# Rose-STL-Lab/spherical-dyffusion

Measured on AMD Instinct MI355X. Metric: forecast-steps/sec (180x360, 63ch), 25-member ensemble DYffusion sampling, whole job, higher is better.
Workload: dtype f32 tensors; every GEMM-class kernel (1x1 convs, fused MLP, Legendre analysis/synthesis, dhconv) as 3-pass split-f16 MFMA with f32 accumulation; FFT / norms / pointwise in f32 (statistics f64)

## Files before the change

### spherical-dyffusion_amd/csrc/conv_h3.hip

```cpp
#include <cmath>
#include <cstdlib>
#include <type_traits>
#include <vector>

#include "common.h"

namespace {

constexpr int CE = 256;
constexpr int CTN = 64;
constexpr int CKMAX = 384;
constexpr int CRING = 4;
constexpr float CSX = SDY_ACT_SX;
constexpr int CSTAT_BYTES = CE * 2 * 8;
#ifndef SDY_CONV_STAMP_T0
#define SDY_CONV_STAMP_T0 2
#endif

template <int KBLK, int NW>
struct ConvCfg {
  static_assert(NW == 4 || NW == 8, "4 or 8 waves");
  static constexpr int NT = 64 * NW;
  static constexpr int MT = 8 / NW;
  static constexpr int RS = 4 * NW;
  static constexpr int OC = (8 * KBLK + RS - 1) / RS;
  static constexpr int RPT = 64 / NW;
  static constexpr int PPI = (8 * OC + RPT - 1) / RPT;
  static constexpr int KROW = KBLK <= 4 ? 256 : 384;
  static constexpr int KSW = KROW / 16;
  static constexpr int GPK = 4 * MT;
  static constexpr int GPW = MT * KSW;
  static constexpr int WGS = NW == 4 ? 2 : 1;
  static constexpr int TILE_BYTES = 2 * CTN * KROW * 2;
  static constexpr int LDS_BYTES = TILE_BYTES + CSTAT_BYTES + CE * 4 + SDY_GELU_TAB_BYTES;
};
#ifndef SDY_CONV_GELU_TAB
#define SDY_CONV_GELU_TAB 1
#endif

struct ConvParams {
  const float* x; long x_bs;
  const float* pa; const float* pd;
  const sdy_f16x8* w;
  const float* bias;
  const float* add; long add_bs; int add_mode;
  int act;
  float* out; long out_bs;
  int out_tiled;
  double* stats;
  int HW, B;
  int Cin;
  float out_scale;
  unsigned* flags;
  unsigned* head;
  const float* gelu_tab;
  SdyImgMap xmap;
  unsigned long long* stamps;
};

__device__ __forceinline__ int cv_swz(int px) { return (px & 15) ^ (((px >> 4) & 1) * 3); }
template <int KROW>
__device__ __forceinline__ int cv_off(int px, int c) { return px * KROW + (((c & ~15) | ((c ^ cv_swz(px)) & 15)) << 3); }

template <int KBLK, int NW>
__global__ __launch_bounds__(64 * NW, NW == 4 ? 2 : 1) void conv_h3_kernel(const ConvParams p) {
  using G = ConvCfg<KBLK, NW>;
  constexpr int CMT = G::MT, CRS = G::RS, COC = G::OC, CRPT = G::RPT, KROW = G::KROW, CGPK = G::GPK, CGPW = G::GPW;
  __shared__ __attribute__((aligned(16))) unsigned char smem[G::LDS_BYTES];
  _Float16* Xs_hi = reinterpret_cast<_Float16*>(smem);
  _Float16* Xs_lo = Xs_hi + CTN * KROW;
  float* Os = reinterpret_cast<float*>(smem);

  const int tid = threadIdx.x, lane = tid & 63, wave = tid >> 6;
  int h = lane >> 5, l31 = lane & 31;
  int q0 = tid & 15, o0 = tid >> 4;
  const int tpi = (p.HW + CTN - 1) / CTN;
  const int ntiles = tpi * p.B;
  const int t_per = (ntiles + (int)gridDim.x - 1) / (int)gridDim.x;
  const int t_begin = (int)blockIdx.x * t_per;
  const int t_end = (t_begin + t_per < ntiles) ? t_begin + t_per : ntiles;

  sdy_f16x8 r_hi[CRING], r_lo[CRING];
  constexpr int CGROUP_BYTES = SDY_GROUP * (int)sizeof(sdy_f16x8);
  const char* const wbase = reinterpret_cast<const char*>(p.w) + (size_t)__builtin_amdgcn_readfirstlane(wave) * CGPW * CGROUP_BYTES;
  unsigned woff = (unsigned)lane * 16u;
#pragma unroll
  for (int s = 0; s < CRING; ++s) {
    r_hi[s] = sdy_ring_ld(wbase, woff, 0);
    r_lo[s] = sdy_ring_ld(wbase, woff, CGROUP_BYTES / 2);
    woff += CGROUP_BYTES;
  }
  constexpr int NWIN = KBLK * CMT;
  if (NWIN == 1) woff -= CRING * CGROUP_BYTES;

  double* Ss = reinterpret_cast<double*>(smem + G::TILE_BYTES);
  float* Bs = reinterpret_cast<float*>(smem + G::TILE_BYTES + CSTAT_BYTES);
  if (tid < CE) {
    Bs[tid] = p.bias ? p.bias[tid] / p.out_scale : 0.0f;
    Ss[2 * tid] = 0.0; Ss[2 * tid + 1] = 0.0;
  }
  float* Gt = reinterpret_cast<float*>(smem + G::TILE_BYTES + CSTAT_BYTES + CE * 4);
  const unsigned gt_base = (unsigned)(uintptr_t)Gt;
  const bool tab_gelu = SDY_CONV_GELU_TAB && p.act == 1;
  if (tab_gelu) gelu_tab_to_lds(Gt, p.gelu_tab, tid, G::NT, 1.0f / SDY_GELU_SX);
  const float os_scale = tab_gelu ? p.out_scale * SDY_GELU_WS : p.out_scale;

  f32x4 xr[COC][8], addv[CRPT];
  auto img = [&](const float* base, long bs, int t) { return base + (long)(t / tpi) * bs; };
  auto ximg = [&](int t) { return p.x + (long)sdy_img(p.xmap, t / tpi) * p.x_bs; };
  auto lane_col = [&](int t) {
    const int nn = (t % tpi) * CTN + 4 * q0;
    return nn < p.HW ? nn : 0;
  };
  const float* addsrc = p.add ? p.add : p.out;
  const long addsrc_bs = p.add ? p.add_bs : p.out_bs;
  if (t_begin < t_end) {
    const float* xz = ximg(t_begin);
    const unsigned xo = (unsigned)(8 * o0 * p.HW + lane_col(t_begin)) * 4u;
#pragma unroll
    for (int oc = 0; oc < COC; ++oc)
#pragma unroll
      for (int e = 0; e < 8; ++e) {
        const int ch = 8 * (o0 + CRS * oc) + e;
        xr[oc][e] = f32x4{0.f, 0.f, 0.f, 0.f};
        if (ch < p.Cin) xr[oc][e] = sdy_ld16s(xz + (long)(8 * CRS * oc + e) * p.HW, xo);
      }
  }

  for (int tile = t_begin; tile < t_end; ++tile) {
    asm volatile("" : "+v"(l31), "+v"(h), "+v"(q0), "+v"(o0));
    const int tile_it = tile - t_begin;
    auto stamp = [&](int i) {
      if (SDY_STAMPS_ON && p.stamps && blockIdx.x == 3 && tid == 0 && tile_it >= SDY_CONV_STAMP_T0 && tile_it < SDY_CONV_STAMP_T0 + 4)
        p.stamps[(tile_it - SDY_CONV_STAMP_T0) * 8 + i] = __builtin_amdgcn_s_memtime();
    };
    stamp(0);
    const int z = tile / tpi;
    const int zx = sdy_img(p.xmap, z);
    const int n0 = (tile - z * tpi) * CTN;
    const bool full = n0 + CTN <= p.HW;

    {
      float amax = 0.0f;
      const bool ok = full || (n0 + 4 * q0 < p.HW);
#pragma unroll
      for (int oc = 0; oc < COC; ++oc) {
        const int c0 = 8 * (o0 + CRS * oc);
        if (8 * CRS * oc + 8 * CRS > KROW && c0 >= KROW) continue;
        float av[8], dv[8];
        if (p.pa) {
          const f32x4 a0 = *reinterpret_cast<const f32x4*>(p.pa + (long)zx * CE + c0);
          const f32x4 a1 = *reinterpret_cast<const f32x4*>(p.pa + (long)zx * CE + c0 + 4);
          const f32x4 d0 = *reinterpret_cast<const f32x4*>(p.pd + (long)zx * CE + c0);
          const f32x4 d1 = *reinterpret_cast<const f32x4*>(p.pd + (long)zx * CE + c0 + 4);
#pragma unroll
          for (int e = 0; e < 4; ++e) {
            av[e] = a0[e] * CSX; av[e + 4] = a1[e] * CSX;
            dv[e] = d0[e] * CSX; dv[e + 4] = d1[e] * CSX;
          }
        } else {
#pragma unroll
          for (int e = 0; e < 8; ++e) { av[e] = CSX; dv[e] = 0.f; }
        }
#pragma unroll
        for (int pp = 0; pp < 4; ++pp) {
          sdy_f16x8 vh, vl;
          float v[8];
#pragma unroll
          for (int e = 0; e < 8; ++e) v[e] = (ok && c0 + e < p.Cin) ? fmaf(xr[oc][e][pp], av[e], dv[e]) : 0.0f;
          sdy_split8(v, vh, vl, amax);
          const int off = cv_off<KROW>(4 * q0 + pp, o0 + CRS * oc);
          *reinterpret_cast<sdy_f16x8*>(Xs_hi + off) = vh;
          *reinterpret_cast<sdy_f16x8*>(Xs_lo + off) = vl;
        }
      }
      sdy_flag_range(p.flags, amax, p.head);
    }
    __syncthreads();
    stamp(1);
    const int col = n0 + 4 * q0;
    const bool c_ok = full || col < p.HW;
    const unsigned ro = (unsigned)(o0 * p.HW + (c_ok ? col : 0)) * 4u;
    const unsigned ro_out = p.out_tiled ? (unsigned)(o0 * CTN + 4 * q0) * 4u : ro;
    const int out_rs = p.out_tiled ? CTN : p.HW;
    const int tnext = (tile + 1 < t_end) ? tile + 1 : tile;
    const float* xz_next = ximg(tnext);
    const unsigned xo_next = (unsigned)(8 * o0 * p.HW + lane_col(tnext)) * 4u;
    stamp(2);
    f32x16 acc[CMT][2];
#pragma unroll
    for (int mi = 0; mi < CMT; ++mi)
#pragma unroll
      for (int r4 = 0; r4 < 4; ++r4) {
        const f32x4 b4 = *reinterpret_cast<const f32x4*>(Bs + 32 * (CMT * wave + mi) + 8 * r4 + 4 * h);
#pragma unroll
        for (int j = 0; j < 2; ++j)
#pragma unroll
          for (int r = 0; r < 4; ++r) acc[mi][j][4 * r4 + r] = b4[r];
      }
#pragma unroll
    for (int kb = 0; kb < KBLK; ++kb) {
#pragma unroll
      for (int i = 0; i < 4; ++i) {
        const int ks = 4 * kb + i;
        sdy_f16x8 bh[2], bl[2];
#pragma unroll
        for (int j = 0; j < 2; ++j) {
          const int off = cv_off<KROW>(32 * j + l31, 2 * ks + h);
          bh[j] = *reinterpret_cast<const sdy_f16x8*>(Xs_hi + off);
          bl[j] = *reinterpret_cast<const sdy_f16x8*>(Xs_lo + off);
        }
#pragma unroll
        for (int mi = 0; mi < CMT; ++mi) {
          const int g = kb * CGPK + CMT * i + mi;
          const int s = g % CRING;
#pragma unroll
          for (int j = 0; j < 2; ++j) SDY_CROSS_TERM(acc[mi][j] = __builtin_amdgcn_mfma_f32_32x32x16_f16(r_lo[s], bh[j], acc[mi][j], 0, 0, 0));
#pragma unroll
          for (int j = 0; j < 2; ++j) SDY_CROSS_TERM(acc[mi][j] = __builtin_amdgcn_mfma_f32_32x32x16_f16(r_hi[s], bl[j], acc[mi][j], 0, 0, 0));
#pragma unroll
          for (int j = 0; j < 2; ++j) acc[mi][j] = __builtin_amdgcn_mfma_f32_32x32x16_f16(r_hi[s], bh[j], acc[mi][j], 0, 0, 0);
          r_hi[s] = sdy_ring_ld(wbase, woff, 0);
          r_lo[s] = sdy_ring_ld(wbase, woff, CGROUP_BYTES / 2);
          woff += CGROUP_BYTES;
          if ((g + CRING + 1) % (NWIN * CRING) == 0) woff -= NWIN * CRING * CGROUP_BYTES;
          __builtin_amdgcn_sched_barrier(0);
        }
      }
    }

    stamp(3);
    {
      const float* az = img(addsrc, addsrc_bs, tile);
#pragma unroll
      for (int i = 0; i < CRPT; ++i) addv[i] = p.add ? sdy_ld16s(az + (long)(CRS * i) * p.HW, ro) : f32x4{0.f, 0.f, 0.f, 0.f};
    }
    __syncthreads();
    stamp(4);
#pragma unroll
    for (int mi = 0; mi < CMT; ++mi)
#pragma unroll
      for (int j = 0; j < 2; ++j)
#pragma unroll
        for (int r = 0; r < 16; ++r) {
          const int row = 32 * (CMT * wave + mi) + (r & 3) + 8 * (r >> 2) + 4 * h;
          Os[row * CTN + 32 * j + l31] = acc[mi][j][r] * os_scale;
        }
    __syncthreads();
    stamp(5);
    {
      float* oz = p.out + (long)z * p.out_bs + (p.out_tiled ? (long)(tile - z * tpi) * (CE * CTN) : 0L);
#pragma unroll
      for (int i = 0; i < CRPT; ++i) {
        f32x4 v = *reinterpret_cast<const f32x4*>(Os + (o0 + CRS * i) * CTN + 4 * q0);
        if (tab_gelu) {
          if (p.add_mode == 1) v = addv[i] * SDY_GELU_WS + v;
          v = f32x4{gelu_tab16(v.x, gt_base), gelu_tab16(v.y, gt_base), gelu_tab16(v.z, gt_base), gelu_tab16(v.w, gt_base)};
        } else {
        if (p.add_mode == 1) v += addv[i];
        if (p.act == 1) {
          const sdy_gf2 g0 = gelu_erf2(sdy_gf2{v.x, v.y}), g1 = gelu_erf2(sdy_gf2{v.z, v.w});
          v = f32x4{g0.x, g0.y, g1.x, g1.y};
        }
        }
        if (p.add_mode == 2) v += addv[i];
        if (c_ok) sdy_st16s(oz + (long)(CRS * i) * out_rs, ro_out, v);
#pragma unroll
        for (int k = 0; k < G::PPI; ++k) {
          const int piece = G::PPI * i + k, oc = piece >> 3, e = piece & 7;
          if (oc < COC) {
            const int ch = 8 * (o0 + CRS * oc) + e;
            if (ch < p.Cin) xr[oc][e] = sdy_ld16s(xz_next + (long)(8 * CRS * oc + e) * p.HW, xo_next);
          }
        }
        if (p.stats) {
          const float s1 = row16_sum(c_ok ? (v.x + v.y) + (v.z + v.w) : 0.0f);
          const float s2 = row16_sum(c_ok ? (v.x * v.x + v.y * v.y) + (v.z * v.z + v.w * v.w) : 0.0f);
          if (q0 == 0) {
            double* st = Ss + 2 * (o0 + CRS * i);
            __hip_atomic_fetch_add(st, (double)s1, __ATOMIC_RELAXED, __HIP_MEMORY_SCOPE_WORKGROUP);
            __hip_atomic_fetch_add(st + 1, (double)s2, __ATOMIC_RELAXED, __HIP_MEMORY_SCOPE_WORKGROUP);
          }
        }
      }
    }
    stamp(6);
    {
      const int nt = tile + 1;
      if (p.stats && (nt >= t_end || nt / tpi != z)) {
        __syncthreads();
        if (tid < CE) {
          double* st = p.stats + ((long)z * CE + tid) * 2;
          __hip_atomic_fetch_add(st, Ss[2 * tid], __ATOMIC_RELAXED, __HIP_MEMORY_SCOPE_AGENT);
          __hip_atomic_fetch_add(st + 1, Ss[2 * tid + 1], __ATOMIC_RELAXED, __HIP_MEMORY_SCOPE_AGENT);
          Ss[2 * tid] = 0.0; Ss[2 * tid + 1] = 0.0;
        }
      }
    }
    stamp(7);
    __syncthreads();
  }
}

}

#if SDY_STAMPS_ON
static unsigned long long* g_cstamps = nullptr;
SDY_DEBUG_EXPORT int sdy_conv256_h3_debug_stamps(unsigned long long* host64) {
  if (!g_cstamps || !host64) return SDY_ERR_STATE;
  SDY_HIP_TRY(hipDeviceSynchronize());
  SDY_HIP_TRY(hipMemcpy(host64, g_cstamps, 64 * sizeof(unsigned long long), hipMemcpyDeviceToHost));
  return SDY_OK;
}
#endif

extern "C" int sdy_conv256_h3_supported(int Cin, int Cout) { return (Cin >= 1 && Cin <= CKMAX && Cout == CE) ? 1 : 0; }

static void conv_layout(int Cin, int* nw, int* ksw, int* mt) {
  const int kblk = (Cin + 63) / 64;
  *nw = kblk <= 4 ? 4 : 8;
  *ksw = kblk <= 4 ? 16 : 24;
  *mt = 8 / *nw;
}

extern "C" size_t sdy_conv256_h3_pack_bytes_cin(int Cin) {
  int nw, ksw, mt;
  conv_layout(Cin < 1 ? 1 : Cin, &nw, &ksw, &mt);
  return (size_t)nw * mt * ksw * SDY_GROUP * sizeof(sdy_f16x8);
}
extern "C" size_t sdy_conv256_h3_pack_bytes(void) { return sdy_conv256_h3_pack_bytes_cin(CE); }

extern "C" int sdy_conv256_h3_pack_cin(const float* w_host, int Cin, void* dev, float* scale) {
  if (!w_host || !dev || !scale || Cin < 1 || Cin > CKMAX) return SDY_ERR_ARG;
  const float s = sdy_h3_scale(sdy_h3_absmax(w_host, (size_t)CE * Cin));
  int nw, ksw, mt;
  conv_layout(Cin, &nw, &ksw, &mt);
  const size_t gh = (size_t)SDY_GROUP * 8;
  std::vector<_Float16> buf((size_t)nw * mt * ksw * gh);
  _Float16* d = buf.data();
  for (int w = 0; w < nw; ++w)
    for (int ks = 0; ks < ksw; ++ks)
      for (int mi = 0; mi < mt; ++mi, d += gh)
        sdy_h3_put_group(d, s, [&](int r, int k) {
          const int kk = 16 * ks + k;
          return kk < Cin ? w_host[(size_t)(32 * (mt * w + mi) + r) * Cin + kk] : 0.0f;
        });
  SDY_HIP_TRY(hipMemcpy(dev, buf.data(), buf.size() * sizeof(_Float16), hipMemcpyHostToDevice));
  *scale = s;
  return SDY_OK;
}
extern "C" int sdy_conv256_h3_pack(const float* w_host, void* dev, float* scale) {
  return sdy_conv256_h3_pack_cin(w_host, CE, dev, scale);
}

template <int KBLK, int NW>
static void conv_launch(const ConvParams& p, long ntiles, int n_cu, hipStream_t stream) {
  using G = ConvCfg<KBLK, NW>;
  const long want = (long)n_cu * G::WGS;
  dim3 grid((unsigned)(ntiles < want ? ntiles : want));
  hipLaunchKernelGGL((conv_h3_kernel<KBLK, NW>), grid, dim3(G::NT), 0, stream, p);
}

int sdy_conv256_h3_launch(const sdy_conv_args* a, hipStream_t stream) {
  if (!a || !a->x || !a->w_frag || !a->out || a->B <= 0 || a->HW <= 0) return SDY_ERR_ARG;
  if (!sdy_conv256_h3_supported(a->Cin, a->Cout)) return SDY_ERR_UNSUPPORTED;
  if (a->drop_p > 0.f || a->keep_mask || a->batch_scale) return SDY_ERR_UNSUPPORTED;
  if (a->pa && a->Cin != CE) return SDY_ERR_UNSUPPORTED;
  if ((a->HW & 3) || (a->x_bstride & 3) || (a->out_bstride & 3) || (a->add_mode && (a->add_bstride & 3))) return SDY_ERR_ALIGN;
  if ((long)a->HW * CKMAX * 4 >= (1L << 32)) return SDY_ERR_UNSUPPORTED;
  ConvParams p;
  p.x = a->x; p.x_bs = a->x_bstride; p.pa = a->pa; p.pd = a->pd;
  p.w = reinterpret_cast<const sdy_f16x8*>(a->w_frag);
  p.bias = a->bias;
  p.add = a->add_mode ? a->add : nullptr; p.add_bs = a->add_bstride; p.add_mode = a->add_mode;
  p.act = a->act;
  p.out = a->out; p.out_bs = a->out_bstride; p.out_tiled = a->out_tiled;
  if (a->out_tiled && a->add_mode && a->add == a->out) return SDY_ERR_ARG;
  p.stats = a->stats;
  SDY_TRY(sdy_flags_ptr(&p.flags));
  SDY_TRY(sdy_headroom_ptr(SDY_RANGE_CONV, &p.head));
  SDY_TRY(sdy_gelu_table_ptr(&p.gelu_tab));
  p.HW = a->HW; p.B = a->B; p.Cin = a->Cin;
  SDY_TRY(sdy_img_map_fill(p.xmap, a->x_rows, a->B));
  p.out_scale = 1.0f / (a->w_frag_scale * CSX);
  p.stamps = nullptr;
#if SDY_STAMPS_ON
  if (std::getenv("SDY_CONV_STAMPS")) {
    if (!g_cstamps) SDY_HIP_TRY(hipMalloc(&g_cstamps, 64 * sizeof(unsigned long long)));
    p.stamps = g_cstamps;
  }
#endif
  int n_cu = 0;
  SDY_TRY(sdy_cu_count(&n_cu));
  const long ntiles = (long)((a->HW + CTN - 1) / CTN) * a->B;
  switch ((a->Cin + 63) / 64) {
    case 1: conv_launch<1, 4>(p, ntiles, n_cu, stream); break;
    case 2: conv_launch<2, 4>(p, ntiles, n_cu, stream); break;
    case 3: conv_launch<3, 4>(p, ntiles, n_cu, stream); break;
    case 4: conv_launch<4, 4>(p, ntiles, n_cu, stream); break;
    case 5: conv_launch<5, 8>(p, ntiles, n_cu, stream); break;
    default: conv_launch<6, 8>(p, ntiles, n_cu, stream); break;
  }
  return sdy_launch_status();
}
```

### spherical-dyffusion_amd/ops.py

```python
from __future__ import annotations

import ctypes as C
from typing import Optional

import torch

from ._lib import SdyConvArgs, SdyMlpArgs, SdyPairArgs, aligned, check, current_stream, lib, ptr


def _f32c(t: torch.Tensor) -> torch.Tensor:
    if not t.is_cuda:
        raise RuntimeError("sdy_amd ops run on the GPU only (no CPU fallback)")
    return aligned(t.to(torch.float32).contiguous())


def _aux(t: torch.Tensor, dev) -> torch.Tensor:
    return t.detach().to(dev, torch.float32).contiguous()


def contract_dhconv(x: torch.Tensor, weight: torch.Tensor, separable: bool = False,
                    operator_type: str = "dhconv", gemm_mode: Optional[str] = None) -> torch.Tensor:
    if separable or operator_type != "dhconv":
        raise NotImplementedError("only the non-separable dhconv contraction is on the hot path")
    B, Ci, L, M = x.shape
    Co = weight.shape[1]
    assert weight.shape == (Ci, Co, L, 2), f"weight shape {tuple(weight.shape)}"
    mtr = min(M, L)
    xr = torch.view_as_real(x.to(torch.complex64).contiguous())
    cs_in = xr[:, :, :, :mtr].permute(2, 3, 0, 4, 1).contiguous()
    cs_out = torch.zeros(L, mtr, B, 2, Co, dtype=torch.float32, device=x.device)
    w_host = weight.detach().to(torch.float32).cpu().contiguous()
    from ._lib import default_gemm_mode
    with torch.cuda.device(x.device):
        mode = gemm_mode or default_gemm_mode()
        if mode == "h3" and lib.sdy_dhconv_frag_supported(Ci, Co):
            wp = torch.empty(lib.sdy_dhconv_frag_pack_bytes(L), dtype=torch.uint8, device=x.device)
            sc = C.c_float()
            check(lib.sdy_dhconv_frag_pack(ptr(w_host), L, ptr(wp), C.byref(sc)), "sdy_dhconv_frag_pack")
            check(lib.sdy_dhconv_frag(ptr(cs_in), ptr(wp), sc.value, ptr(cs_out), L, mtr, B, current_stream()),
                  "sdy_dhconv_frag")
        elif mode == "h3":
            wp = torch.empty(lib.sdy_dhconv_h3_pack_bytes(Ci, Co, L), dtype=torch.uint8, device=x.device)
            sc = C.c_float()
            check(lib.sdy_dhconv_h3_pack_weight(ptr(w_host), Ci, Co, L, ptr(wp), C.byref(sc)), "sdy_dhconv_h3_pack_weight")
            check(lib.sdy_dhconv_h3(ptr(cs_in), ptr(wp), sc.value, ptr(cs_out), L, mtr, B, Ci, Co, current_stream()),
                  "sdy_dhconv_h3")
        else:
            wp = torch.empty(L * 2 * Ci * Co, dtype=torch.float32, device=x.device)
            check(lib.sdy_dhconv_pack_weight(ptr(w_host), Ci, Co, L, ptr(wp), current_stream()), "sdy_dhconv_pack_weight")
            check(lib.sdy_dhconv(ptr(cs_in), ptr(wp), ptr(cs_out), L, mtr, B, Ci, Co, current_stream()), "sdy_dhconv")
    out = torch.zeros(B, Co, L, M, 2, dtype=torch.float32, device=x.device)
    out[:, :, :, :mtr] = cs_out.permute(2, 4, 0, 1, 3)
    tri = (torch.arange(M, device=x.device)[None, :] <= torch.arange(L, device=x.device)[:, None])
    out = out * tri[None, None, :, :, None]
    return torch.view_as_complex(out.contiguous())


def instnorm_coeffs(x: torch.Tensor, gamma: torch.Tensor, beta: torch.Tensor,
                    scale_shift: Optional[torch.Tensor] = None, eps: float = 1e-6):
    x = _f32c(x)
    B, Cc, H, W = x.shape
    a = torch.empty(B, Cc, dtype=torch.float32, device=x.device)
    d = torch.empty_like(a)
    g, b_ = _aux(gamma, x.device), _aux(beta, x.device)
    ss = _aux(scale_shift, x.device) if scale_shift is not None else None
    with torch.cuda.device(x.device):
        check(lib.sdy_instnorm_coeffs(ptr(x), B, Cc, H * W, ptr(g), ptr(b_), ptr(ss), 2 * Cc, eps, ptr(a), ptr(d),
                                      current_stream()), "sdy_instnorm_coeffs")
    return a, d


def conv1x1(x: torch.Tensor, weight: torch.Tensor, bias: Optional[torch.Tensor] = None, *,
            pre_affine=None, add: Optional[torch.Tensor] = None, add_mode: int = 0, gelu: bool = False,
            drop_p: float = 0.0, keep_mask: Optional[torch.Tensor] = None, seed: int = 0, call: int = 0,
            stream_id: int = 0, batch_offset: int = 0, batch_scale: Optional[torch.Tensor] = None,
            kernel_tag: int = 0, out: Optional[torch.Tensor] = None, wt_prepared=None, h3: bool = False,
            h3_prepared=None, frag_prepared=None, stats: Optional[torch.Tensor] = None) -> torch.Tensor:
    x = _f32c(x)
    B, Cin, H, W = x.shape
    w2 = weight.detach().to(torch.float32).reshape(weight.shape[0], -1)
    Cout = w2.shape[0]
    assert w2.shape[1] == Cin
    ldw = (Cout + 3) // 4 * 4
    if wt_prepared is not None:
        wt = wt_prepared
    else:
        wt = torch.zeros(Cin, ldw, dtype=torch.float32, device=x.device)
        wt[:, :Cout] = w2.t().to(x.device)
    if out is None:
        out = torch.empty(B, Cout, H, W, dtype=torch.float32, device=x.device)
    a = SdyConvArgs()
    a.x, a.x_bstride = ptr(x), Cin * H * W
    a.wt, a.ldw = ptr(wt), ldw
    a.out, a.out_bstride = ptr(out), Cout * H * W
    a.B, a.Cin, a.Cout, a.HW = B, Cin, Cout, H * W
    keep = [x, wt, out]
    if h3 or h3_prepared is not None:
        if h3_prepared is None:
            h3_prepared = pack_h3(w2, x.device)
        a.w_h3, a.w_h3_scale = ptr(h3_prepared[0]), h3_prepared[1]
        keep.append(h3_prepared[0])
    if pre_affine is not None:
        pa, pd = _aux(pre_affine[0], x.device), _aux(pre_affine[1], x.device)
        a.pa, a.pd = ptr(pa), ptr(pd)
        keep += [pa, pd]
    if bias is not None:
        bb = _aux(bias, x.device)
        a.bias = ptr(bb)
        keep.append(bb)
    if add is not None:
        ad = _aux(add, x.device)
        a.add = ptr(ad)
        a.add_bstride = 0 if ad.shape[0] == 1 and B > 1 else Cout * H * W
        a.add_mode = add_mode
        keep.append(ad)
    a.act = 1 if gelu else 0
    a.drop_p = drop_p
    if keep_mask is not None:
        km = _aux(keep_mask, x.device)
        a.keep_mask = ptr(km)
        keep.append(km)
    a.seed, a.call, a.stream_id, a.batch_offset = seed, call, stream_id, batch_offset
    a.kernel_tag = kernel_tag
    if frag_prepared is not None:
        a.w_frag, a.w_frag_scale = ptr(frag_prepared[0]), frag_prepared[1]
        keep.append(frag_prepared[0])
    if stats is not None:
        assert stats.dtype == torch.float64 and stats.is_cuda and stats.is_contiguous() and stats.numel() == B * Cout * 2
        a.stats = ptr(stats)
    if batch_scale is not None:
        bs = _aux(batch_scale, x.device)
        a.batch_scale = ptr(bs)
        keep.append(bs)
    with torch.cuda.device(x.device):
        check(lib.sdy_conv1x1(C.byref(a), current_stream()), "sdy_conv1x1")
    return out


def pack_conv256(weight: torch.Tensor, device):
    w = weight.detach().to("cpu", torch.float32).reshape(weight.shape[0], -1).contiguous()
    if not lib.sdy_conv256_h3_supported(w.shape[1], w.shape[0]):
        raise NotImplementedError("the persistent conv kernel needs 256 output and at most 384 input channels")
    buf = torch.empty(lib.sdy_conv256_h3_pack_bytes_cin(w.shape[1]), dtype=torch.uint8, device=device)
    sc = C.c_float()
    with torch.cuda.device(device):
        check(lib.sdy_conv256_h3_pack_cin(ptr(w), w.shape[1], ptr(buf), C.byref(sc)), "sdy_conv256_h3_pack_cin")
    return buf, sc.value


def pack_h3(weight: torch.Tensor, device):
    w = weight.detach().to("cpu", torch.float32).reshape(weight.shape[0], -1).contiguous()
    Cout, Cin = w.shape
    nbytes = lib.sdy_h3_pack_bytes(Cout, Cin)
    buf = torch.empty(nbytes, dtype=torch.uint8, device=device)
    sc = C.c_float()
    with torch.cuda.device(device):
        check(lib.sdy_h3_pack_weight(ptr(w), Cout, Cin, ptr(buf), C.byref(sc)), "sdy_h3_pack_weight")
    return buf, sc.value


def pack_mlp_h3(w1: torch.Tensor, w2: torch.Tensor, device):
    a = w1.detach().to("cpu", torch.float32).reshape(w1.shape[0], -1).contiguous()
    b = w2.detach().to("cpu", torch.float32).reshape(w2.shape[0], -1).contiguous()
    hidden, E = a.shape
    assert b.shape == (E, hidden)
    if not lib.sdy_mlp_h3_supported(E, hidden):
        raise NotImplementedError(f"fused MLP kernel supports E=256, hidden=512 (got {E}, {hidden}); use conv1x1")
    buf = torch.empty(lib.sdy_mlp_h3_pack_bytes(E, hidden), dtype=torch.uint8, device=device)
    s1, s2 = C.c_float(), C.c_float()
    with torch.cuda.device(device):
        check(lib.sdy_mlp_h3_pack(ptr(a), ptr(b), E, hidden, ptr(buf), C.byref(s1), C.byref(s2)), "sdy_mlp_h3_pack")
    return (buf, s1.value, s2.value)


def mlp_fused(x: torch.Tensor, w1: torch.Tensor, b1: torch.Tensor, w2: torch.Tensor, b2: torch.Tensor, *,
              pre_affine=None, add: Optional[torch.Tensor] = None, drop_p: float = 0.0, seed: int = 0, call: int = 0,
              stream_fc1: int = 0, stream_fc2: int = 1, batch_offset: int = 0,
              batch_scale: Optional[torch.Tensor] = None, out: Optional[torch.Tensor] = None,
              prepared=None, add_affine=None, stats: Optional[torch.Tensor] = None,
              keep_masks=None) -> torch.Tensor:
    x = _f32c(x)
    B, E, H, W = x.shape
    if prepared is None:
        prepared = pack_mlp_h3(w1, w2, x.device)
    hidden = b1.numel()
    if out is None:
        out = torch.empty_like(x)
    a = SdyMlpArgs()
    a.x, a.x_bstride = ptr(x), E * H * W
    a.w, a.w1_scale, a.w2_scale = ptr(prepared[0]), prepared[1], prepared[2]
    bb1, bb2 = _aux(b1, x.device), _aux(b2, x.device)
    a.b1, a.b2 = ptr(bb1), ptr(bb2)
    a.out, a.out_bstride = ptr(out), E * H * W
    keep = [x, bb1, bb2, out, prepared]
    if pre_affine is not None:
        pa, pd = _aux(pre_affine[0], x.device), _aux(pre_affine[1], x.device)
        a.pa, a.pd = ptr(pa), ptr(pd)
        keep += [pa, pd]
    if add is not None:
        ad = _aux(add, x.device)
        a.add, a.add_bstride = ptr(ad), E * H * W
        keep.append(ad)
        if add_affine is not None:
            ra, rd = _aux(add_affine[0], x.device), _aux(add_affine[1], x.device)
            a.add_a, a.add_d = ptr(ra), ptr(rd)
            keep += [ra, rd]
    a.B, a.E, a.hidden, a.HW = B, E, hidden, H * W
    a.drop_p = drop_p
    a.seed, a.call, a.stream_fc1, a.stream_fc2, a.batch_offset = seed, call, stream_fc1, stream_fc2, batch_offset
    if batch_scale is not None:
        bs = _aux(batch_scale, x.device)
        a.batch_scale = ptr(bs)
        keep.append(bs)
    if stats is not None:
        assert stats.dtype == torch.float64 and stats.is_cuda and stats.is_contiguous() and stats.numel() == B * E * 2
        a.stats = ptr(stats)
    if keep_masks is not None:
        kh, ko = _aux(keep_masks[0], x.device), _aux(keep_masks[1], x.device)
        assert kh.numel() == B * hidden * H * W and ko.numel() == B * E * H * W
        a.keep_hidden, a.keep_out = ptr(kh), ptr(ko)
        keep += [kh, ko]
    with torch.cuda.device(x.device):
        check(lib.sdy_mlp_h3(C.byref(a), current_stream()), "sdy_mlp_h3")
    return out


def pack_pair_h3(w1: torch.Tensor, w2: torch.Tensor, device):
    a = w1.detach().to("cpu", torch.float32).reshape(w1.shape[0], -1).contiguous()
    b = w2.detach().to("cpu", torch.float32).reshape(w2.shape[0], -1).contiguous()
    hidden, Cin = a.shape
    Cout = b.shape[0]
    assert b.shape == (Cout, hidden)
    if not lib.sdy_pair_h3_supported(Cin, hidden, Cout):
        raise NotImplementedError(f"fused conv pair supports hidden=256 with (Cin<=144, Cout=256) or (Cin<=416, Cout<=64); "
                                  f"got {Cin}->{hidden}->{Cout}; use conv1x1 twice")
    buf = torch.empty(lib.sdy_pair_h3_pack_bytes(Cin, hidden, Cout), dtype=torch.uint8, device=device)
    s1, s2 = C.c_float(), C.c_float()
    with torch.cuda.device(device):
        check(lib.sdy_pair_h3_pack(ptr(a), ptr(b), Cin, hidden, Cout, ptr(buf), C.byref(s1), C.byref(s2)), "sdy_pair_h3_pack")
    return (buf, s1.value, s2.value)


def conv_pair(x: torch.Tensor, w1: torch.Tensor, b1: Optional[torch.Tensor], w2: torch.Tensor, *,
              add: Optional[torch.Tensor] = None, out: Optional[torch.Tensor] = None, prepared=None,
              stats: Optional[torch.Tensor] = None) -> torch.Tensor:
    x = _f32c(x)
    B, Cin, H, W = x.shape
    if prepared is None:
        prepared = pack_pair_h3(w1, w2, x.device)
    hidden, Cout = w1.shape[0], w2.shape[0]
    if out is None:
        out = torch.empty(B, Cout, H, W, dtype=torch.float32, device=x.device)
    a = SdyPairArgs()
    a.x, a.x_bstride = ptr(x), Cin * H * W
    a.w, a.w1_scale, a.w2_scale = ptr(prepared[0]), prepared[1], prepared[2]
    keep = [x, out, prepared]
    if b1 is not None:
        bb1 = _aux(b1, x.device)
        a.b1 = ptr(bb1)
        keep.append(bb1)
    a.out, a.out_bstride = ptr(out), Cout * H * W
    if add is not None:
        ad = _aux(add, x.device)
        a.add, a.add_bstride = ptr(ad), (0 if ad.shape[0] == 1 and B > 1 else Cout * H * W)
        keep.append(ad)
    a.B, a.Cin, a.hidden, a.Cout, a.HW = B, Cin, hidden, Cout, H * W
    if stats is not None:
        assert stats.dtype == torch.float64 and stats.is_cuda and stats.is_contiguous() and stats.numel() == B * Cout * 2
        a.stats = ptr(stats)
    with torch.cuda.device(x.device):
        check(lib.sdy_pair_h3(C.byref(a), current_stream()), "sdy_pair_h3")
    return out


def instnorm_from_stats(stats: torch.Tensor, HW: int, gamma: torch.Tensor, beta: torch.Tensor, scale_shift=None,
                        eps: float = 1e-6):
    B, Cc = stats.shape[0], stats.shape[1]
    dev = stats.device
    g, b_ = _aux(gamma, dev), _aux(beta, dev)
    ss = _aux(scale_shift, dev) if scale_shift is not None else None
    a = torch.empty(B, Cc, dtype=torch.float32, device=dev)
    d = torch.empty(B, Cc, dtype=torch.float32, device=dev)
    with torch.cuda.device(dev):
        check(lib.sdy_instnorm_from_stats(ptr(stats), B, Cc, HW, ptr(g), ptr(b_), ptr(ss), 2 * Cc if ss is not None else 0,
                                          eps, ptr(a), ptr(d), current_stream()), "sdy_instnorm_from_stats")
    return a, d


def cold_update(x_s: torch.Tensor, x_ip_next: torch.Tensor, x_ip_s: Optional[torch.Tensor]) -> torch.Tensor:
    a, b = _f32c(x_s), _f32c(x_ip_next)
    c = _f32c(x_ip_s) if x_ip_s is not None else None
    out = torch.empty_like(a)
    with torch.cuda.device(a.device):
        check(lib.sdy_cold_update(ptr(a), ptr(b), ptr(c), ptr(out), a.numel(), current_stream()), "sdy_cold_update")
    return out


def concat_channels(tensors) -> torch.Tensor:
    ts = [_f32c(t) for t in tensors]
    if len(ts) == 1:
        return ts[0]
    assert 1 <= len(ts) <= 4
    B, _, H, W = ts[0].shape
    chans = [t.shape[1] for t in ts]
    out = torch.empty(B, sum(chans), H, W, dtype=torch.float32, device=ts[0].device)
    srcs = (C.c_void_p * len(ts))(*[ptr(t) for t in ts])
    ch = (C.c_int * len(ts))(*chans)
    with torch.cuda.device(out.device):
        check(lib.sdy_concat_channels(srcs, ch, len(ts), ptr(out), B, H * W, current_stream()), "sdy_concat_channels")
    return out


FLAG_NONFINITE, FLAG_F16_RANGE = 1, 2


def status_flags(reset: bool = True, device=None) -> int:
    dev = torch.device("cuda", torch.cuda.current_device()) if device is None else torch.device(device)
    out = C.c_uint(0)
    with torch.cuda.device(dev):
        check(lib.sdy_status_flags(C.byref(out), 1 if reset else 0, current_stream()), "sdy_status_flags")
    return int(out.value)


RANGE_CLASSES = ("conv_h3 x tile", "mlp_h3 x tile", "dh_h3 coefficient rows", "Legendre analysis input (at rfft360's stores)",
                 "Legendre synthesis input (at dh_h3's stores)")


class range_headroom:

    LIMIT = 65504.0

    def __enter__(self):
        buf = (C.c_float * len(RANGE_CLASSES))()
        with torch.cuda.device(torch.cuda.current_device()):
            check(lib.sdy_range_headroom(buf, 1, current_stream()), "sdy_range_headroom")
        check(lib.sdy_range_headroom_enable(1))
        self.max_staged, self.factor = {}, {}
        return self

    def __exit__(self, *exc):
        check(lib.sdy_range_headroom_enable(0))
        buf = (C.c_float * len(RANGE_CLASSES))()
        with torch.cuda.device(torch.cuda.current_device()):
            check(lib.sdy_range_headroom(buf, 1, current_stream()), "sdy_range_headroom")
        self.max_staged = {n: float(buf[i]) for i, n in enumerate(RANGE_CLASSES)}
        self.factor = {n: (self.LIMIT / v if v > 0.0 else float("inf")) for n, v in self.max_staged.items()}
        return False


def raise_on_status_flags(flags: int, where: str) -> None:
    if not flags:
        return
    why = []
    if flags & FLAG_F16_RANGE:
        why.append("an activation exceeded the fp16 range of the split-precision kernels (|value| * 16 >= 65504, i.e. "
                   "|value| >= 4094 after normalisation)")
    if flags & FLAG_NONFINITE:
        why.append("an InstanceNorm statistic came out inf / NaN (a tensor inside the network holds non-finite values)")
    from ._lib import SdyError
    raise SdyError(f"{where}: " + "; ".join(why) + ".  Inputs are expected standardised; if the data really need the range, "
                   "run the fp32-MFMA path: SDY_GEMM_MODE=f32 (or gemm_mode='f32').")


class stage_timer:

    def __enter__(self):
        n = lib.sdy_profile_stage_count()
        check(lib.sdy_profile_read((C.c_double * n)(), (C.c_long * n)(), n))
        check(lib.sdy_profile_enable(1))
        self.stages, self.rows = {}, {}
        return self

    def __exit__(self, *exc):
        check(lib.sdy_profile_enable(0))
        n = lib.sdy_profile_stage_count()
        ms, cnt, rows = (C.c_double * n)(), (C.c_long * n)(), (C.c_long * n)()
        check(lib.sdy_profile_read_rows(ms, cnt, rows, n), "sdy_profile_read_rows")
        self.stages = {lib.sdy_profile_stage_name(i).decode(): (int(cnt[i]), float(ms[i])) for i in range(n) if cnt[i]}
        self.rows = {lib.sdy_profile_stage_name(i).decode(): int(rows[i]) for i in range(n) if cnt[i]}
        return False
```

Baseline: 162.5.

## Split conv K-staging and epilogue into halves to fit three workgroups per CU

Sets the 4-wave conv kernel's occupancy target to 3 workgroups per CU and halves the LDS x-tile. The input is staged and consumed in two K halves with a barrier between them, and the fp32 epilogue is written out in two row halves. This cuts LDS footprint and register pressure so more waves can hide latency. In exchange it adds extra barriers and serialises staging against the MFMA work within a tile. The Python wrapper also gains out_tiled and x_rows options.

```diff
diff --git a/spherical-dyffusion_amd/csrc/conv_h3.hip b/spherical-dyffusion_amd/csrc/conv_h3.hip
--- a/spherical-dyffusion_amd/csrc/conv_h3.hip
+++ b/spherical-dyffusion_amd/csrc/conv_h3.hip
@@ -13,6 +13,9 @@
 constexpr int CRING = 4;
 constexpr float CSX = SDY_ACT_SX;
 constexpr int CSTAT_BYTES = CE * 2 * 8;
+#ifndef SDY_CONV_WGS
+#define SDY_CONV_WGS 3
+#endif
 #ifndef SDY_CONV_STAMP_T0
 #define SDY_CONV_STAMP_T0 2
 #endif
@@ -25,13 +28,21 @@
   static constexpr int RS = 4 * NW;
   static constexpr int OC = (8 * KBLK + RS - 1) / RS;
   static constexpr int RPT = 64 / NW;
-  static constexpr int PPI = (8 * OC + RPT - 1) / RPT;
   static constexpr int KROW = KBLK <= 4 ? 256 : 384;
   static constexpr int KSW = KROW / 16;
   static constexpr int GPK = 4 * MT;
   static constexpr int GPW = MT * KSW;
-  static constexpr int WGS = NW == 4 ? 2 : 1;
-  static constexpr int TILE_BYTES = 2 * CTN * KROW * 2;
+  static constexpr int WGS = NW == 4 ? SDY_CONV_WGS : 1;
+  static constexpr int NSP = WGS >= 3 ? 2 : 1;
+  static_assert(NSP == 1 || (NSP == MT && KROW == 256 && RS == KROW / 8 / NSP), "halves = the staging role's octet sets");
+  static constexpr int KH = KROW / NSP;
+  static constexpr int KBH = KROW / 64 / NSP;
+  static constexpr int NKH = (KBLK + KBH - 1) / KBH;
+  static constexpr int RPR = RPT / NSP;
+  static constexpr int PPI = (8 * OC + RPT - 1) / RPT;
+  static constexpr int row_c(int rd, int i) { return NSP == 1 ? RS * i : 32 * (MT * ((RS * i) >> 5) + rd) + ((RS * i) & 31); }
+  static constexpr int TILE_BYTES = 2 * CTN * KH * 2;
+  static_assert(CE / NSP * CTN * 4 <= TILE_BYTES, "the epilogue's fp32 staging aliases the x tile");
   static constexpr int LDS_BYTES = TILE_BYTES + CSTAT_BYTES + CE * 4 + SDY_GELU_TAB_BYTES;
 };
 #ifndef SDY_CONV_GELU_TAB
@@ -58,22 +69,36 @@
   unsigned long long* stamps;
 };
 
+__device__ __forceinline__ float sdy_uniform(float v) {
+  return __builtin_bit_cast(float, __builtin_amdgcn_readfirstlane(__builtin_bit_cast(int, v)));
+}
 __device__ __forceinline__ int cv_swz(int px) { return (px & 15) ^ (((px >> 4) & 1) * 3); }
 template <int KROW>
 __device__ __forceinline__ int cv_off(int px, int c) { return px * KROW + (((c & ~15) | ((c ^ cv_swz(px)) & 15)) << 3); }
 
 template <int KBLK, int NW>
-__global__ __launch_bounds__(64 * NW, NW == 4 ? 2 : 1) void conv_h3_kernel(const ConvParams p) {
+__global__ __launch_bounds__(64 * NW, NW == 4 ? SDY_CONV_WGS : 1) void conv_h3_kernel(const ConvParams p) {
   using G = ConvCfg<KBLK, NW>;
-  constexpr int CMT = G::MT, CRS = G::RS, COC = G::OC, CRPT = G::RPT, KROW = G::KROW, CGPK = G::GPK, CGPW = G::GPW;
+  constexpr int CMT = G::MT, CRS = G::RS, COC = G::OC, KROW = G::KROW, CGPK = G::GPK, CGPW = G::GPW;
+  constexpr int NSP = G::NSP, KH = G::KH, KBH = G::KBH, NKH = G::NKH, RPR = G::RPR;
   __shared__ __attribute__((aligned(16))) unsigned char smem[G::LDS_BYTES];
   _Float16* Xs_hi = reinterpret_cast<_Float16*>(smem);
-  _Float16* Xs_lo = Xs_hi + CTN * KROW;
+  _Float16* Xs_lo = Xs_hi + CTN * KH;
   float* Os = reinterpret_cast<float*>(smem);
 
-  const int tid = threadIdx.x, lane = tid & 63, wave = tid >> 6;
+  const int tid = threadIdx.x, lane = tid & 63;
+  const int wave = __builtin_amdgcn_readfirstlane(tid >> 6);
   int h = lane >> 5, l31 = lane & 31;
   int q0 = tid & 15, o0 = tid >> 4;
+  int tl = tid;
+  auto fence_ids = [&]() {
+    if (NSP > 1) {
+      asm volatile("" : "+v"(tl));
+      l31 = tl & 31; h = (tl >> 5) & 1; q0 = tl & 15; o0 = tl >> 4;
+    } else {
+      asm volatile("" : "+v"(l31), "+v"(h), "+v"(q0), "+v"(o0));
+    }
+  };
   const int tpi = (p.HW + CTN - 1) / CTN;
   const int ntiles = tpi * p.B;
   const int t_per = (ntiles + (int)gridDim.x - 1) / (int)gridDim.x;
@@ -82,7 +107,7 @@
 
   sdy_f16x8 r_hi[CRING], r_lo[CRING];
   constexpr int CGROUP_BYTES = SDY_GROUP * (int)sizeof(sdy_f16x8);
-  const char* const wbase = reinterpret_cast<const char*>(p.w) + (size_t)__builtin_amdgcn_readfirstlane(wave) * CGPW * CGROUP_BYTES;
+  const char* const wbase = reinterpret_cast<const char*>(p.w) + (size_t)wave * CGPW * CGROUP_BYTES;
   unsigned woff = (unsigned)lane * 16u;
 #pragma unroll
   for (int s = 0; s < CRING; ++s) {
@@ -103,11 +128,11 @@
   const unsigned gt_base = (unsigned)(uintptr_t)Gt;
   const bool tab_gelu = SDY_CONV_GELU_TAB && p.act == 1;
   if (tab_gelu) gelu_tab_to_lds(Gt, p.gelu_tab, tid, G::NT, 1.0f / SDY_GELU_SX);
-  const float os_scale = tab_gelu ? p.out_scale * SDY_GELU_WS : p.out_scale;
-
-  f32x4 xr[COC][8], addv[CRPT];
+  const float os_scale = sdy_uniform(tab_gelu ? p.out_scale * SDY_GELU_WS : p.out_scale);
+
+  f32x4 xr[COC][8], addv[RPR];
   auto img = [&](const float* base, long bs, int t) { return base + (long)(t / tpi) * bs; };
-  auto ximg = [&](int t) { return p.x + (long)sdy_img(p.xmap, t / tpi) * p.x_bs; };
+  auto ximg = [&](int t) { return p.x + (long)__builtin_amdgcn_readfirstlane(sdy_img(p.xmap, t / tpi)) * p.x_bs; };
   auto lane_col = [&](int t) {
     const int nn = (t % tpi) * CTN + 4 * q0;
     return nn < p.HW ? nn : 0;
@@ -128,7 +153,7 @@
   }
 
   for (int tile = t_begin; tile < t_end; ++tile) {
-    asm volatile("" : "+v"(l31), "+v"(h), "+v"(q0), "+v"(o0));
+    fence_ids();
     const int tile_it = tile - t_begin;
     auto stamp = [&](int i) {
       if (SDY_STAMPS_ON && p.stamps && blockIdx.x == 3 && tid == 0 && tile_it >= SDY_CONV_STAMP_T0 && tile_it < SDY_CONV_STAMP_T0 + 4)
@@ -140,44 +165,124 @@
     const int n0 = (tile - z * tpi) * CTN;
     const bool full = n0 + CTN <= p.HW;
 
-    {
-      float amax = 0.0f;
-      const bool ok = full || (n0 + 4 * q0 < p.HW);
-#pragma unroll
-      for (int oc = 0; oc < COC; ++oc) {
-        const int c0 = 8 * (o0 + CRS * oc);
-        if (8 * CRS * oc + 8 * CRS > KROW && c0 >= KROW) continue;
-        float av[8], dv[8];
-        if (p.pa) {
-          const f32x4 a0 = *reinterpret_cast<const f32x4*>(p.pa + (long)zx * CE + c0);
-          const f32x4 a1 = *reinterpret_cast<const f32x4*>(p.pa + (long)zx * CE + c0 + 4);
-          const f32x4 d0 = *reinterpret_cast<const f32x4*>(p.pd + (long)zx * CE + c0);
-          const f32x4 d1 = *reinterpret_cast<const f32x4*>(p.pd + (long)zx * CE + c0 + 4);
-#pragma unroll
-          for (int e = 0; e < 4; ++e) {
-            av[e] = a0[e] * CSX; av[e + 4] = a1[e] * CSX;
-            dv[e] = d0[e] * CSX; dv[e + 4] = d1[e] * CSX;
-          }
-        } else {
-#pragma unroll
-          for (int e = 0; e < 8; ++e) { av[e] = CSX; dv[e] = 0.f; }
-        }
-#pragma unroll
-        for (int pp = 0; pp < 4; ++pp) {
-          sdy_f16x8 vh, vl;
-          float v[8];
-#pragma unroll
-          for (int e = 0; e < 8; ++e) v[e] = (ok && c0 + e < p.Cin) ? fmaf(xr[oc][e][pp], av[e], dv[e]) : 0.0f;
-          sdy_split8(v, vh, vl, amax);
-          const int off = cv_off<KROW>(4 * q0 + pp, o0 + CRS * oc);
-          *reinterpret_cast<sdy_f16x8*>(Xs_hi + off) = vh;
-          *reinterpret_cast<sdy_f16x8*>(Xs_lo + off) = vl;
-        }
-      }
-      sdy_flag_range(p.flags, amax, p.head);
+    f32x16 acc[CMT][2];
+#pragma unroll
+    for (int hf = 0; hf < NKH; ++hf) {
+      if (hf > 0) __syncthreads();
+      {
+        float amax = 0.0f;
+        const bool ok = full || (n0 + 4 * q0 < p.HW);
+#pragma unroll
+        for (int oc = 0; oc < COC; ++oc) {
+          if (NSP > 1 && oc != hf) continue;
+          const int c0 = 8 * (o0 + CRS * oc);
+          if (8 * CRS * oc + 8 * CRS > KROW && c0 >= KROW) continue;
+          if (NSP > 1) {
+#pragma unroll
+            for (int e = 0; e < 8; ++e) {
+              const float a = p.pa ? p.pa[(long)zx * CE + c0 + e] * CSX : CSX;
+              const float d = p.pa ? p.pd[(long)zx * CE + c0 + e] * CSX : 0.f;
+              const bool on = ok && c0 + e < p.Cin;
+#pragma unroll
+              for (int pp = 0; pp < 4; ++pp) xr[oc][e][pp] = on ? fmaf(xr[oc][e][pp], a, d) : 0.0f;
+            }
+#pragma unroll
+            for (int pp = 0; pp < 4; ++pp) {
+              sdy_f16x8 vh, vl;
+              float v[8];
+#pragma unroll
+              for (int e = 0; e < 8; ++e) v[e] = xr[oc][e][pp];
+              sdy_split8(v, vh, vl, amax);
+              const int off = cv_off<KH>(4 * q0 + pp, o0);
+              *reinterpret_cast<sdy_f16x8*>(Xs_hi + off) = vh;
+              *reinterpret_cast<sdy_f16x8*>(Xs_lo + off) = vl;
+              __builtin_amdgcn_sched_barrier(0);
+            }
+            continue;
+          }
+          float av[8], dv[8];
+          if (p.pa) {
+            const f32x4 a0 = *reinterpret_cast<const f32x4*>(p.pa + (long)zx * CE + c0);
+            const f32x4 a1 = *reinterpret_cast<const f32x4*>(p.pa + (long)zx * CE + c0 + 4);
+            const f32x4 d0 = *reinterpret_cast<const f32x4*>(p.pd + (long)zx * CE + c0);
+            const f32x4 d1 = *reinterpret_cast<const f32x4*>(p.pd + (long)zx * CE + c0 + 4);
+#pragma unroll
+            for (int e = 0; e < 4; ++e) {
+              av[e] = a0[e] * CSX; av[e + 4] = a1[e] * CSX;
+              dv[e] = d0[e] * CSX; dv[e + 4] = d1[e] * CSX;
+            }
+          } else {
+#pragma unroll
+            for (int e = 0; e < 8; ++e) { av[e] = CSX; dv[e] = 0.f; }
+          }
+#pragma unroll
+          for (int pp = 0; pp < 4; ++pp) {
+            sdy_f16x8 vh, vl;
+            float v[8];
+#pragma unroll
+            for (int e = 0; e < 8; ++e) v[e] = (ok && c0 + e < p.Cin) ? fmaf(xr[oc][e][pp], av[e], dv[e]) : 0.0f;
+            sdy_split8(v, vh, vl, amax);
+            const int off = cv_off<KH>(4 * q0 + pp, o0 + CRS * oc);
+            *reinterpret_cast<sdy_f16x8*>(Xs_hi + off) = vh;
+            *reinterpret_cast<sdy_f16x8*>(Xs_lo + off) = vl;
+          }
+        }
+        sdy_flag_range(p.flags, amax, p.head);
+      }
+      __syncthreads();
+      if (NSP > 1) fence_ids();
+      if (hf == 0) {
+        stamp(1);
+        stamp(2);
+#pragma unroll
+        for (int mi = 0; mi < CMT; ++mi)
+#pragma unroll
+          for (int r4 = 0; r4 < 4; ++r4) {
+            const f32x4 b4 = *reinterpret_cast<const f32x4*>(Bs + 32 * (CMT * wave + mi) + 8 * r4 + 4 * h);
+#pragma unroll
+            for (int j = 0; j < 2; ++j)
+#pragma unroll
+              for (int r = 0; r < 4; ++r) acc[mi][j][4 * r4 + r] = b4[r];
+          }
+      }
+#pragma unroll
+      for (int kb = hf * KBH; kb < (hf + 1) * KBH; ++kb) {
+        if (kb >= KBLK) continue;
+#pragma unroll
+        for (int i = 0; i < 4; ++i) {
+          const int ks = 4 * kb + i;
+          sdy_f16x8 bh[2], bl[2];
+#pragma unroll
+          for (int j = 0; j < 2; ++j) {
+            const int off = cv_off<KH>(32 * j + l31, 2 * (ks - hf * (KH / 16)) + h);
+            bh[j] = *reinterpret_cast<const sdy_f16x8*>(Xs_hi + off);
+            bl[j] = *reinterpret_cast<const sdy_f16x8*>(Xs_lo + off);
+          }
+#pragma unroll
+          for (int mi = 0; mi < CMT; ++mi) {
+            const int g = kb * CGPK + CMT * i + mi;
+            const int s = g % CRING;
+#pragma unroll
+            for (int j = 0; j < 2; ++j) SDY_CROSS_TERM(acc[mi][j] = __builtin_amdgcn_mfma_f32_32x32x16_f16(r_lo[s], bh[j], acc[mi][j], 0, 0, 0));
+#pragma unroll
+            for (int j = 0; j < 2; ++j) SDY_CROSS_TERM(acc[mi][j] = __builtin_amdgcn_mfma_f32_32x32x16_f16(r_hi[s], bl[j], acc[mi][j], 0, 0, 0));
+#pragma unroll
+            for (int j = 0; j < 2; ++j) acc[mi][j] = __builtin_amdgcn_mfma_f32_32x32x16_f16(r_hi[s], bh[j], acc[mi][j], 0, 0, 0);
+#ifndef SDY_CONV_NO_REFILL_FENCE
+            if (NSP > 1) __builtin_amdgcn_sched_barrier(0);
+#endif
+            r_hi[s] = sdy_ring_ld(wbase, woff, 0);
+            r_lo[s] = sdy_ring_ld(wbase, woff, CGROUP_BYTES / 2);
+            woff += CGROUP_BYTES;
+            if ((g + CRING + 1) % (NWIN * CRING) == 0) woff -= NWIN * CRING * CGROUP_BYTES;
+            __builtin_amdgcn_sched_barrier(0);
+          }
+        }
+      }
     }
-    __syncthreads();
-    stamp(1);
+
+    stamp(3);
+    if (NSP > 1) fence_ids();
     const int col = n0 + 4 * q0;
     const bool c_ok = full || col < p.HW;
     const unsigned ro = (unsigned)(o0 * p.HW + (c_ok ? col : 0)) * 4u;
@@ -186,72 +291,33 @@
     const int tnext = (tile + 1 < t_end) ? tile + 1 : tile;
     const float* xz_next = ximg(tnext);
     const unsigned xo_next = (unsigned)(8 * o0 * p.HW + lane_col(tnext)) * 4u;
-    stamp(2);
-    f32x16 acc[CMT][2];
-#pragma unroll
-    for (int mi = 0; mi < CMT; ++mi)
-#pragma unroll
-      for (int r4 = 0; r4 < 4; ++r4) {
-        const f32x4 b4 = *reinterpret_cast<const f32x4*>(Bs + 32 * (CMT * wave + mi) + 8 * r4 + 4 * h);
-#pragma unroll
-        for (int j = 0; j < 2; ++j)
-#pragma unroll
-          for (int r = 0; r < 4; ++r) acc[mi][j][4 * r4 + r] = b4[r];
-      }
-#pragma unroll
-    for (int kb = 0; kb < KBLK; ++kb) {
-#pragma unroll
-      for (int i = 0; i < 4; ++i) {
-        const int ks = 4 * kb + i;
-        sdy_f16x8 bh[2], bl[2];
+    const float* az = img(addsrc, addsrc_bs, tile);
+    {
+#pragma unroll
+      for (int i = 0; i < RPR; ++i) addv[i] = p.add ? sdy_ld16s(az + (long)G::row_c(0, i) * p.HW, ro) : f32x4{0.f, 0.f, 0.f, 0.f};
+    }
+    float* oz = p.out + (long)z * p.out_bs + (p.out_tiled ? (long)(tile - z * tpi) * (CE * CTN) : 0L);
+#pragma unroll
+    for (int rd = 0; rd < NSP; ++rd) {
+      __syncthreads();
+      if (rd == 0) stamp(4);
+#pragma unroll
+      for (int mi = 0; mi < CMT; ++mi) {
+        if (NSP > 1 && mi != rd) continue;
 #pragma unroll
         for (int j = 0; j < 2; ++j) {
-          const int off = cv_off<KROW>(32 * j + l31, 2 * ks + h);
-          bh[j] = *reinterpret_cast<const sdy_f16x8*>(Xs_hi + off);
-          bl[j] = *reinterpret_cast<const sdy_f16x8*>(Xs_lo + off);
-        }
-#pragma unroll
-        for (int mi = 0; mi < CMT; ++mi) {
-          const int g = kb * CGPK + CMT * i + mi;
-          const int s = g % CRING;
-#pragma unroll
-          for (int j = 0; j < 2; ++j) SDY_CROSS_TERM(acc[mi][j] = __builtin_amdgcn_mfma_f32_32x32x16_f16(r_lo[s], bh[j], acc[mi][j], 0, 0, 0));
-#pragma unroll
-          for (int j = 0; j < 2; ++j) SDY_CROSS_TERM(acc[mi][j] = __builtin_amdgcn_mfma_f32_32x32x16_f16(r_hi[s], bl[j], acc[mi][j], 0, 0, 0));
-#pragma unroll
-          for (int j = 0; j < 2; ++j) acc[mi][j] = __builtin_amdgcn_mfma_f32_32x32x16_f16(r_hi[s], bh[j], acc[mi][j], 0, 0, 0);
-          r_hi[s] = sdy_ring_ld(wbase, woff, 0);
-          r_lo[s] = sdy_ring_ld(wbase, woff, CGROUP_BYTES / 2);
-          woff += CGROUP_BYTES;
-          if ((g + CRING + 1) % (NWIN * CRING) == 0) woff -= NWIN * CRING * CGROUP_BYTES;
-          __builtin_amdgcn_sched_barrier(0);
-        }
-      }
-    }
-
-    stamp(3);
-    {
-      const float* az = img(addsrc, addsrc_bs, tile);
-#pragma unroll
-      for (int i = 0; i < CRPT; ++i) addv[i] = p.add ? sdy_ld16s(az + (long)(CRS * i) * p.HW, ro) : f32x4{0.f, 0.f, 0.f, 0.f};
-    }
-    __syncthreads();
-    stamp(4);
-#pragma unroll
-    for (int mi = 0; mi < CMT; ++mi)
-#pragma unroll
-      for (int j = 0; j < 2; ++j)
-#pragma unroll
-        for (int r = 0; r < 16; ++r) {
-          const int row = 32 * (CMT * wave + mi) + (r & 3) + 8 * (r >> 2) + 4 * h;
-          Os[row * CTN + 32 * j + l31] = acc[mi][j][r] * os_scale;
-        }
-    __syncthreads();
-    stamp(5);
-    {
-      float* oz = p.out + (long)z * p.out_bs + (p.out_tiled ? (long)(tile - z * tpi) * (CE * CTN) : 0L);
-#pragma unroll
-      for (int i = 0; i < CRPT; ++i) {
+#pragma unroll
+          for (int r = 0; r < 16; ++r) {
+            const int row = 32 * (NSP > 1 ? wave : CMT * wave + mi) + (r & 3) + 8 * (r >> 2) + 4 * h;
+            Os[row * CTN + 32 * j + l31] = acc[mi][j][r] * os_scale;
+          }
+        }
+      }
+      __syncthreads();
+      if (rd == 0) stamp(5);
+#pragma unroll
+      for (int i = 0; i < RPR; ++i) {
+        const int rc = G::row_c(rd, i);
         f32x4 v = *reinterpret_cast<const f32x4*>(Os + (o0 + CRS * i) * CTN + 4 * q0);
         if (tab_gelu) {
           if (p.add_mode == 1) v = addv[i] * SDY_GELU_WS + v;
@@ -264,20 +330,31 @@
         }
         }
         if (p.add_mode == 2) v += addv[i];
-        if (c_ok) sdy_st16s(oz + (long)(CRS * i) * out_rs, ro_out, v);
-#pragma unroll
+        if (c_ok) sdy_st16s(oz + (long)rc * out_rs, ro_out, v);
+#pragma unroll
+#ifdef SDY_CONV_X_LATE
+        for (int k = 0; k < 2 * G::PPI; ++k) {
+#else
         for (int k = 0; k < G::PPI; ++k) {
-          const int piece = G::PPI * i + k, oc = piece >> 3, e = piece & 7;
+#endif
+#ifdef SDY_CONV_X_LATE
+          const int piece = 2 * G::PPI * i + k, oc = piece >> 3, e = piece & 7;
+          if (rd == NSP - 1 && oc < COC) {
+#else
+          const int piece = G::PPI * (RPR * rd + i) + k, oc = piece >> 3, e = piece & 7;
           if (oc < COC) {
+#endif
             const int ch = 8 * (o0 + CRS * oc) + e;
+            if (NSP > 1) xr[oc][e] = f32x4{0.f, 0.f, 0.f, 0.f};
             if (ch < p.Cin) xr[oc][e] = sdy_ld16s(xz_next + (long)(8 * CRS * oc + e) * p.HW, xo_next);
           }
         }
+        if (rd + 1 < NSP && p.add) addv[i] = sdy_ld16s(az + (long)G::row_c(rd + 1, i) * p.HW, ro);
         if (p.stats) {
           const float s1 = row16_sum(c_ok ? (v.x + v.y) + (v.z + v.w) : 0.0f);
           const float s2 = row16_sum(c_ok ? (v.x * v.x + v.y * v.y) + (v.z * v.z + v.w * v.w) : 0.0f);
           if (q0 == 0) {
-            double* st = Ss + 2 * (o0 + CRS * i);
+            double* st = Ss + 2 * (o0 + rc);
             __hip_atomic_fetch_add(st, (double)s1, __ATOMIC_RELAXED, __HIP_MEMORY_SCOPE_WORKGROUP);
             __hip_atomic_fetch_add(st + 1, (double)s2, __ATOMIC_RELAXED, __HIP_MEMORY_SCOPE_WORKGROUP);
           }
@@ -289,11 +366,19 @@
       const int nt = tile + 1;
       if (p.stats && (nt >= t_end || nt / tpi != z)) {
         __syncthreads();
-        if (tid < CE) {
-          double* st = p.stats + ((long)z * CE + tid) * 2;
-          __hip_atomic_fetch_add(st, Ss[2 * tid], __ATOMIC_RELAXED, __HIP_MEMORY_SCOPE_AGENT);
-          __hip_atomic_fetch_add(st + 1, Ss[2 * tid + 1], __ATOMIC_RELAXED, __HIP_MEMORY_SCOPE_AGENT);
-          Ss[2 * tid] = 0.0; Ss[2 * tid + 1] = 0.0;
+        fence_ids();
+        const int ft = NSP > 1 ? tl : tid;
+        if (ft < CE) {
+          double* st = p.stats + ((long)z * CE + ft) * 2;
+          __hip_atomic_fetch_add(st, Ss[2 * ft], __ATOMIC_RELAXED, __HIP_MEMORY_SCOPE_AGENT);
+          __hip_atomic_fetch_add(st + 1, Ss[2 * ft + 1], __ATOMIC_RELAXED, __HIP_MEMORY_SCOPE_AGENT);
+          if (NSP > 1) {
+            int zi = 0;
+            asm volatile("" : "+v"(zi));
+            *reinterpret_cast<int4*>(Ss + 2 * ft) = int4{zi, zi, zi, zi};
+          } else {
+            Ss[2 * ft] = 0.0; Ss[2 * ft + 1] = 0.0;
+          }
         }
       }
     }
diff --git a/spherical-dyffusion_amd/ops.py b/spherical-dyffusion_amd/ops.py
--- a/spherical-dyffusion_amd/ops.py
+++ b/spherical-dyffusion_amd/ops.py
@@ -75,9 +75,13 @@
             drop_p: float = 0.0, keep_mask: Optional[torch.Tensor] = None, seed: int = 0, call: int = 0,
             stream_id: int = 0, batch_offset: int = 0, batch_scale: Optional[torch.Tensor] = None,
             kernel_tag: int = 0, out: Optional[torch.Tensor] = None, wt_prepared=None, h3: bool = False,
-            h3_prepared=None, frag_prepared=None, stats: Optional[torch.Tensor] = None) -> torch.Tensor:
+            h3_prepared=None, frag_prepared=None, stats: Optional[torch.Tensor] = None,
+            out_tiled: bool = False, x_rows=None) -> torch.Tensor:
     x = _f32c(x)
     B, Cin, H, W = x.shape
+    if x_rows is not None:
+        B = len(x_rows)
+    keep = []
     w2 = weight.detach().to(torch.float32).reshape(weight.shape[0], -1)
     Cout = w2.shape[0]
     assert w2.shape[1] == Cin
@@ -88,13 +92,19 @@
         wt = torch.zeros(Cin, ldw, dtype=torch.float32, device=x.device)
         wt[:, :Cout] = w2.t().to(x.device)
     if out is None:
-        out = torch.empty(B, Cout, H, W, dtype=torch.float32, device=x.device)
+        shape = (B, (H * W + 63) // 64, Cout, 64) if out_tiled else (B, Cout, H, W)
+        out = torch.empty(shape, dtype=torch.float32, device=x.device)
     a = SdyConvArgs()
     a.x, a.x_bstride = ptr(x), Cin * H * W
     a.wt, a.ldw = ptr(wt), ldw
-    a.out, a.out_bstride = ptr(out), Cout * H * W
+    a.out, a.out_bstride = ptr(out), out[0].numel()
+    a.out_tiled = 1 if out_tiled else 0
+    if x_rows is not None:
+        rows = (C.c_ubyte * B)(*[int(r) for r in x_rows])
+        a.x_rows = C.cast(rows, C.c_void_p)
+        keep.append(rows)
     a.B, a.Cin, a.Cout, a.HW = B, Cin, Cout, H * W
-    keep = [x, wt, out]
+    keep += [x, wt, out]
     if h3 or h3_prepared is not None:
         if h3_prepared is None:
             h3_prepared = pack_h3(w2, x.device)
```

After: 162.3. About the same (-0.1%).
